# adityaX1412/Experiment-YOLO

Hardware: AMD Instinct MI355X
Metric: images/sec (train) DEAL-YOLO-N 640x640 bs=64/GPU (higher is better)
Workload: dtype f16; 1 GPU; DEAL-YOLO-N (yolov8n-ASF-P2P2.yaml) train step 640x640, per-GPU batch 64, fwd+TAL/WIOU+NWD/DFL/BCE loss+bwd+SGD+EMA, BASELINE.json configs[1]; loss_mode=wiou+nwd, settle_steps=18, capture_retries=0, global_batch=64, parallelism=dp1, hipgraph=True

## Files before the change

### experiment-yolo_amd/csrc/tensor_ops.hip

```cpp
#include <cstdlib>
#include "common.h"
#include "dealyolo_hip.h"

static inline int grid_for(long total) {
  long b = (total + 255) / 256;
  if (b > 8192) b = 8192;
  if (b < 1) b = 1;
  return (int)b;
}
static bool tensor_ops_v1() {
  const char* e = getenv("DY_TENSOR_OPS_V1");
  return e && e[0] == '1' && !e[1];
}

__global__ __launch_bounds__(256) void import_image_kernel(const float* x, f16* y, int N, int C, int H, int W, int Cp,
                                                           float mul) {
  const long hw = (long)H * W, total = (long)N * hw;
  for (long pix = (long)blockIdx.x * 256 + threadIdx.x; pix < total; pix += (long)gridDim.x * 256) {
    const long n = pix / hw, r = pix - n * hw;
    for (int c0 = 0; c0 < Cp; c0 += 8) {
      half8 v;
#pragma unroll
      for (int j = 0; j < 8; ++j) v[j] = (c0 + j < C) ? (f16)(x[(n * C + c0 + j) * hw + r] * mul) : (f16)0.f;
      *reinterpret_cast<half8*>(y + pix * Cp + c0) = v;
// ... 329 lines not shown
            bi[j] = dy * 5 + dx;
          }
        }
      }
    }
    half8 o;
    uint8_t ai[8];
#pragma unroll
    for (int j = 0; j < 8; ++j) {
      o[j] = (f16)best[j];
      ai[j] = (uint8_t)bi[j];
    }
    *reinterpret_cast<half8*>(a.y + pix * a.ldy + c0) = o;
    if (a.arg) *reinterpret_cast<uint2*>(a.arg + pix * a.C + c0) = *reinterpret_cast<uint2*>(ai);
  }
}
__global__ __launch_bounds__(256) void maxpool5_bwd_kernel(PoolArgs a) {
  const int cpp = a.C >> 3;
  const long total = (long)a.N * a.H * a.W * cpp;
  for (long idx = (long)blockIdx.x * 256 + threadIdx.x; idx < total; idx += (long)gridDim.x * 256) {
    const long pix = idx / cpp;
    const int c0 = (int)(idx - pix * cpp) * 8;
    const int x0 = (int)(pix % a.W);
    const long t = pix / a.W;
    const int y0 = (int)(t % a.H);
    const long n = t / a.H;
    float s[8];
#pragma unroll
    for (int j = 0; j < 8; ++j) s[j] = 0.f;
    if (a.accumulate) {
      const half8 o = *reinterpret_cast<const half8*>(a.y + pix * a.ldy + c0);
#pragma unroll
      for (int j = 0; j < 8; ++j) s[j] = (float)o[j];
    }
#pragma unroll
    for (int dy = 0; dy < 5; ++dy) {
      const int wy = y0 - (dy - 2);
      const bool yok = wy >= 0 && wy < a.H;
      const int yc = yok ? wy : y0;
      uint2 raw[5];
      half8 g[5];
      bool ok[5];
#pragma unroll
      for (int dx = 0; dx < 5; ++dx) {
        const int wx = x0 - (dx - 2);
        ok[dx] = yok && wx >= 0 && wx < a.W;
        const long wp = (n * a.H + yc) * a.W + (ok[dx] ? wx : x0);
        raw[dx] = *reinterpret_cast<const uint2*>(a.arg + wp * a.C + c0);
        g[dx] = *reinterpret_cast<const half8*>(a.dy + wp * a.lddy + c0);
      }
#pragma unroll
      for (int dx = 0; dx < 5; ++dx) {
        if (!ok[dx]) continue;
        const uint8_t* ai = reinterpret_cast<const uint8_t*>(&raw[dx]);
        const int code = dy * 5 + dx;
#pragma unroll
        for (int j = 0; j < 8; ++j)
          if (ai[j] == code) s[j] += (float)g[dx][j];
      }
    }
    half8 o;
#pragma unroll
    for (int j = 0; j < 8; ++j) o[j] = (f16)s[j];
    *reinterpret_cast<half8*>(a.y + pix * a.ldy + c0) = o;
  }
}
#define SPPF_THREADS 1024
struct SppfArgs {
  f16* cat;
  uint8_t* arg[3];
  int ld, C, N, H, W, acc[3];
};
template <int CG>
static __device__ __forceinline__ void sppf_pool3_fwd_body(const SppfArgs& a, char* sppf_lds) {
  constexpr int G = CG / 8;
  const int HW = a.H * a.W, items = HW * G;
  half8* cur = reinterpret_cast<half8*>(sppf_lds);
  half8* rowm = cur + items;
  uint2* rowa = reinterpret_cast<uint2*>(rowm + items);
  const int groups = a.C / CG, n = blockIdx.x / groups, c0 = (blockIdx.x - n * groups) * CG;
  f16* const base = a.cat + (size_t)n * HW * a.ld + c0;
  for (int i = threadIdx.x; i < items; i += SPPF_THREADS) {
    const int px = i / G, part = i - px * G;
    cur[i] = *reinterpret_cast<const half8*>(base + (size_t)px * a.ld + part * 8);
  }
  __syncthreads();
  for (int l = 0; l < 3; ++l) {
    for (int i = threadIdx.x; i < items; i += SPPF_THREADS) {
      const int px = i / G, part = i - px * G, y = px / a.W, x = px - y * a.W;
      float best[8];
      uint8_t bd[8];
#pragma unroll
      for (int j = 0; j < 8; ++j) { best[j] = -INFINITY; bd[j] = 0; }
#pragma unroll
      for (int dx = 0; dx < 5; ++dx) {
        const int xx = x + dx - 2;
        if (xx < 0 || xx >= a.W) continue;
        const half8 v = cur[(y * a.W + xx) * G + part];
#pragma unroll
        for (int j = 0; j < 8; ++j) {
          const float f = (float)v[j];
          if (f > best[j] || f != f) { best[j] = f; bd[j] = (uint8_t)dx; }
        }
      }
      half8 o;
#pragma unroll
      for (int j = 0; j < 8; ++j) o[j] = (f16)best[j];
      rowm[i] = o;
      rowa[i] = *reinterpret_cast<const uint2*>(bd);
    }
    __syncthreads();
    f16* const yb = base + (size_t)(l + 1) * a.C;
    uint8_t* const ab = a.arg[l] ? a.arg[l] + (size_t)n * HW * a.C + c0 : nullptr;
    for (int i = threadIdx.x; i < items; i += SPPF_THREADS) {
      const int px = i / G, part = i - px * G, y = px / a.W, x = px - y * a.W;
      float best[8];
      uint8_t bi[8];
#pragma unroll
      for (int j = 0; j < 8; ++j) { best[j] = -INFINITY; bi[j] = 0; }
#pragma unroll
      for (int dy = 0; dy < 5; ++dy) {
        const int yy = y + dy - 2;
        if (yy < 0 || yy >= a.H) continue;
        const int k = (yy * a.W + x) * G + part;
        const half8 v = rowm[k];
        const uint2 ra = rowa[k];
        const uint8_t* rd = reinterpret_cast<const uint8_t*>(&ra);
#pragma unroll
        for (int j = 0; j < 8; ++j) {
          const float f = (float)v[j];
          if (f > best[j] || f != f) { best[j] = f; bi[j] = (uint8_t)(dy * 5 + rd[j]); }
        }
      }
      half8 o;
#pragma unroll
      for (int j = 0; j < 8; ++j) o[j] = (f16)best[j];
      cur[i] = o;
      *reinterpret_cast<half8*>(yb + (size_t)px * a.ld + part * 8) = o;
      if (ab) *reinterpret_cast<uint2*>(ab + (size_t)px * a.C + part * 8) = *reinterpret_cast<const uint2*>(bi);
    }
    __syncthreads();
  }
}
template <int CG>
__global__ __launch_bounds__(SPPF_THREADS) void sppf_pool3_fwd_kernel(SppfArgs a) {
  extern __shared__ __attribute__((aligned(16))) char sppf_lds[];
  sppf_pool3_fwd_body<CG>(a, sppf_lds);
}
template <int CG>
__global__ __launch_bounds__(SPPF_THREADS) void sppf_pool3_fwd_v2_kernel(SppfArgs a) {
  constexpr int G = CG / 8;
  constexpr unsigned KNINF = 0x03ffu;
  extern __shared__ __attribute__((aligned(16))) char sppf_lds[];
  const int HW = a.H * a.W, items = HW * G;
  uint4* cur = reinterpret_cast<uint4*>(sppf_lds);
  uint4* row0 = cur + items;
  uint4* row1 = row0 + items;
  int* special = reinterpret_cast<int*>(row1 + items);
  const int groups = a.C / CG, n = blockIdx.x / groups, c0 = (blockIdx.x - n * groups) * CG;
  f16* const base = a.cat + (size_t)n * HW * a.ld + c0;
  if (threadIdx.x == 0) *special = 0;
  __syncthreads();
  bool bad = false;
  for (int i = threadIdx.x; i < items; i += SPPF_THREADS) {
    const int px = i / G, part = i - px * G;
    const uint4 v = *reinterpret_cast<const uint4*>(base + (size_t)px * a.ld + part * 8);
    const unsigned w[4] = {v.x, v.y, v.z, v.w};
    unsigned k[4];
#pragma unroll
    for (int d = 0; d < 4; ++d) {
      const unsigned lo = w[d] & 0xffffu, hi = w[d] >> 16;
      bad |= (lo & 0x7fffu) > 0x7c00u || lo == 0x8000u || (hi & 0x7fffu) > 0x7c00u || hi == 0x8000u;
      k[d] = w[d] ^ ((((w[d] >> 15) & 0x00010001u) * 0xffffu) | 0x80008000u);
    }
    cur[i] = uint4{k[0], k[1], k[2], k[3]};
  }
  if (bad) *special = 1;
  __syncthreads();
  if (*special) {
    __syncthreads();
    sppf_pool3_fwd_body<CG>(a, sppf_lds);
    return;
  }
  for (int l = 0; l < 3; ++l) {
    for (int i = threadIdx.x; i < items; i += SPPF_THREADS) {
      const int px = i / G, part = i - px * G, y = px / a.W, x = px - y * a.W;
      unsigned best[8];
#pragma unroll
      for (int dx = 0; dx < 5; ++dx) {
        const int xx = min(max(x + dx - 2, 0), a.W - 1);
        const unsigned t = (unsigned)(63 - xx);
        const uint4 v = cur[(y * a.W + xx) * G + part];
        const unsigned w[4] = {v.x, v.y, v.z, v.w};
#pragma unroll
        for (int d = 0; d < 4; ++d) {
          const unsigned lo = (w[d] << 16) | t, hi = (w[d] & 0xffff0000u) | t;
          best[2 * d] = dx ? max(best[2 * d], lo) : lo;
          best[2 * d + 1] = dx ? max(best[2 * d + 1], hi) : hi;
        }
      }
      const int kx = (63 - y) * 5 + x - 61, ninf = (63 - y) * 5 + 4;
      unsigned o[8];
#pragma unroll
      for (int j = 0; j < 8; ++j) {
        const unsigned low = (best[j] >> 16) == KNINF ? (unsigned)ninf : (unsigned)((int)(best[j] & 0xffffu) + kx);
        o[j] = (best[j] & 0xffff0000u) | low;
      }
      row0[i] = uint4{o[0], o[1], o[2], o[3]};
      row1[i] = uint4{o[4], o[5], o[6], o[7]};
    }
    __syncthreads();
    f16* const yb = base + (size_t)(l + 1) * a.C;
    uint8_t* const ab = a.arg[l] ? a.arg[l] + (size_t)n * HW * a.C + c0 : nullptr;
    for (int i = threadIdx.x; i < items; i += SPPF_THREADS) {
      const int px = i / G, part = i - px * G, y = px / a.W, x = px - y * a.W;
      unsigned best[8];
#pragma unroll
      for (int dy = 0; dy < 5; ++dy) {
        const int yy = min(max(y + dy - 2, 0), a.H - 1);
        const int k = (yy * a.W + x) * G + part;
        const uint4 v0 = row0[k], v1 = row1[k];
        const unsigned w[8] = {v0.x, v0.y, v0.z, v0.w, v1.x, v1.y, v1.z, v1.w};
#pragma unroll
        for (int j = 0; j < 8; ++j) best[j] = dy ? max(best[j], w[j]) : w[j];
      }
      const unsigned ky = (unsigned)(329 - 5 * y);
      unsigned kp[4], hv[4], code[8];
#pragma unroll
      for (int j = 0; j < 8; ++j) code[j] = (best[j] >> 16) == KNINF ? 0u : (ky - (best[j] & 0xffffu)) & 0xffu;
#pragma unroll
      for (int d = 0; d < 4; ++d) {
        kp[d] = (best[2 * d + 1] & 0xffff0000u) | (best[2 * d] >> 16);
        hv[d] = kp[d] ^ ((((~kp[d] >> 15) & 0x00010001u) * 0xffffu) | 0x80008000u);
      }
      cur[i] = uint4{kp[0], kp[1], kp[2], kp[3]};
      *reinterpret_cast<uint4*>(yb + (size_t)px * a.ld + part * 8) = uint4{hv[0], hv[1], hv[2], hv[3]};
      if (ab)
        *reinterpret_cast<uint2*>(ab + (size_t)px * a.C + part * 8) =
            uint2{code[0] | code[1] << 8 | code[2] << 16 | code[3] << 24, code[4] | code[5] << 8 | code[6] << 16 | code[7] << 24};
    }
    __syncthreads();
  }
}
template <int CG>
__global__ __launch_bounds__(SPPF_THREADS) void sppf_pool3_bwd_kernel(SppfArgs a) {
  constexpr int G = CG / 8;
  extern __shared__ __attribute__((aligned(16))) char sppf_lds[];
  const int HW = a.H * a.W, items = HW * G;
  half8* g0 = reinterpret_cast<half8*>(sppf_lds);
  half8* g1 = g0 + items;
  uint2* ar = reinterpret_cast<uint2*>(g1 + items);
  const int groups = a.C / CG, n = blockIdx.x / groups, c0 = (blockIdx.x - n * groups) * CG;
  f16* const base = a.cat + (size_t)n * HW * a.ld + c0;
  for (int i = threadIdx.x; i < items; i += SPPF_THREADS) {
    const int px = i / G, part = i - px * G;
    g0[i] = *reinterpret_cast<const half8*>(base + (size_t)3 * a.C + (size_t)px * a.ld + part * 8);
  }
  for (int l = 2; l >= 0; --l) {
    const uint8_t* const ab = a.arg[l] + (size_t)n * HW * a.C + c0;
    for (int i = threadIdx.x; i < items; i += SPPF_THREADS) {
      const int px = i / G, part = i - px * G;
      ar[i] = *reinterpret_cast<const uint2*>(ab + (size_t)px * a.C + part * 8);
    }
    __syncthreads();
    f16* const tb = base + (size_t)l * a.C;
    for (int i = threadIdx.x; i < items; i += SPPF_THREADS) {
      const int px = i / G, part = i - px * G, y = px / a.W, x = px - y * a.W;
      float s[8];
#pragma unroll
      for (int j = 0; j < 8; ++j) s[j] = 0.f;
      if (a.acc[l]) {
        const half8 o = *reinterpret_cast<const half8*>(tb + (size_t)px * a.ld + part * 8);
#pragma unroll
        for (int j = 0; j < 8; ++j) s[j] = (float)o[j];
      }
#pragma unroll
      for (int dy = 0; dy < 5; ++dy) {
        const int wy = y - (dy - 2);
        if (wy < 0 || wy >= a.H) continue;
#pragma unroll
        for (int dx = 0; dx < 5; ++dx) {
          const int wx = x - (dx - 2);
          if (wx < 0 || wx >= a.W) continue;
          const int k = (wy * a.W + wx) * G + part;
          const uint2 raw = ar[k];
          const half8 g = g0[k];
          const uint8_t* ai = reinterpret_cast<const uint8_t*>(&raw);
          const int code = dy * 5 + dx;
#pragma unroll
          for (int j = 0; j < 8; ++j)
            if (ai[j] == code) s[j] += (float)g[j];
        }
      }
      half8 o;
#pragma unroll
      for (int j = 0; j < 8; ++j) o[j] = (f16)s[j];
      if (l > 0) g1[i] = o;
      else *reinterpret_cast<half8*>(tb + (size_t)px * a.ld + part * 8) = o;
    }
    __syncthreads();
    half8* t = g0; g0 = g1; g1 = t;
  }
}
extern "C" int dy_sppf_pool3_supported(int h, int w, int C) {
  if (h < 1 || w < 1 || C < 8 || (C & 7)) return 0;
  const long px = (long)h * w;
  if (!(C & 15) && px * (2 * 32 + 16) <= 156 * 1024) return 16;
  if (px * (2 * 16 + 8) <= 156 * 1024) return 8;
  return 0;
}
extern "C" int dy_sppf_pool3(void* cat, int ld, int C, void* arg0, void* arg1, void* arg2, int n, int h, int w, hipStream_t stream) {
  const int cg = dy_sppf_pool3_supported(h, w, C);
  if (!cg || !cat || ld < 4 * C) return DY_ERR_ARG;
  if ((ld & 7) || ((uintptr_t)cat & 15)) return DY_ERR_ALIGN;
  SppfArgs a{(f16*)cat, {(uint8_t*)arg0, (uint8_t*)arg1, (uint8_t*)arg2}, ld, C, n, h, w, {0, 0, 0}};
  const size_t lds2 = (size_t)h * w * (cg / 8) * 48 + 16;
  if (!tensor_ops_v1() && h <= 63 && w <= 63 && lds2 <= 156 * 1024) {
    static bool attr2[2] = {false, false};
    if (cg == 16) {
      if (!attr2[0]) { if (hipFuncSetAttribute(reinterpret_cast<const void*>(sppf_pool3_fwd_v2_kernel<16>), hipFuncAttributeMaxDynamicSharedMemorySize, 156 * 1024) != hipSuccess) return DY_ERR_LAUNCH; attr2[0] = true; }
      hipLaunchKernelGGL(sppf_pool3_fwd_v2_kernel<16>, dim3(n * (C / 16)), dim3(SPPF_THREADS), lds2, stream, a);
    } else {
      if (!attr2[1]) { if (hipFuncSetAttribute(reinterpret_cast<const void*>(sppf_pool3_fwd_v2_kernel<8>), hipFuncAttributeMaxDynamicSharedMemorySize, 156 * 1024) != hipSuccess) return DY_ERR_LAUNCH; attr2[1] = true; }
      hipLaunchKernelGGL(sppf_pool3_fwd_v2_kernel<8>, dim3(n * (C / 8)), dim3(SPPF_THREADS), lds2, stream, a);
    }
    DY_CHECK_LAUNCH();
    return DY_OK;
  }
  const size_t lds = (size_t)h * w * (cg / 8) * (2 * 16 + 8);
  static bool attr[2] = {false, false};
  if (cg == 16) {
    if (!attr[0]) { if (hipFuncSetAttribute(reinterpret_cast<const void*>(sppf_pool3_fwd_kernel<16>), hipFuncAttributeMaxDynamicSharedMemorySize, 156 * 1024) != hipSuccess) return DY_ERR_LAUNCH; attr[0] = true; }
    hipLaunchKernelGGL(sppf_pool3_fwd_kernel<16>, dim3(n * (C / 16)), dim3(SPPF_THREADS), lds, stream, a);
  } else {
    if (!attr[1]) { if (hipFuncSetAttribute(reinterpret_cast<const void*>(sppf_pool3_fwd_kernel<8>), hipFuncAttributeMaxDynamicSharedMemorySize, 156 * 1024) != hipSuccess) return DY_ERR_LAUNCH; attr[1] = true; }
    hipLaunchKernelGGL(sppf_pool3_fwd_kernel<8>, dim3(n * (C / 8)), dim3(SPPF_THREADS), lds, stream, a);
  }
  DY_CHECK_LAUNCH();
  return DY_OK;
}
extern "C" int dy_sppf_pool3_backward(void* gcat, int ld, int C, const void* arg0, const void* arg1, const void* arg2, int n, int h,
                                      int w, int acc0, int acc1, int acc2, hipStream_t stream) {
  const int cg = dy_sppf_pool3_supported(h, w, C);
  if (!cg || !gcat || !arg0 || !arg1 || !arg2 || ld < 4 * C) return DY_ERR_ARG;
  if ((ld & 7) || ((uintptr_t)gcat & 15)) return DY_ERR_ALIGN;
  SppfArgs a{(f16*)gcat, {(uint8_t*)arg0, (uint8_t*)arg1, (uint8_t*)arg2}, ld, C, n, h, w, {acc0, acc1, acc2}};
  const size_t lds = (size_t)h * w * (cg / 8) * (2 * 16 + 8);
  static bool attr[2] = {false, false};
  if (cg == 16) {
    if (!attr[0]) { if (hipFuncSetAttribute(reinterpret_cast<const void*>(sppf_pool3_bwd_kernel<16>), hipFuncAttributeMaxDynamicSharedMemorySize, 156 * 1024) != hipSuccess) return DY_ERR_LAUNCH; attr[0] = true; }
    hipLaunchKernelGGL(sppf_pool3_bwd_kernel<16>, dim3(n * (C / 16)), dim3(SPPF_THREADS), lds, stream, a);
  } else {
    if (!attr[1]) { if (hipFuncSetAttribute(reinterpret_cast<const void*>(sppf_pool3_bwd_kernel<8>), hipFuncAttributeMaxDynamicSharedMemorySize, 156 * 1024) != hipSuccess) return DY_ERR_LAUNCH; attr[1] = true; }
    hipLaunchKernelGGL(sppf_pool3_bwd_kernel<8>, dim3(n * (C / 8)), dim3(SPPF_THREADS), lds, stream, a);
  }
  DY_CHECK_LAUNCH();
  return DY_OK;
}

extern "C" int dy_maxpool5(const void* x, int ldx, void* y, int ldy, void* argmax, int n, int h, int w, int C,
                           hipStream_t stream) {
  if ((C & 7) || (ldx & 7) || (ldy & 7)) return DY_ERR_ALIGN;
  PoolArgs a{(const f16*)x, (f16*)y, (uint8_t*)argmax, nullptr, ldx, ldy, 0, C, n, h, w, 0};
  hipLaunchKernelGGL(maxpool5_fwd_kernel, dim3(grid_for((long)n * h * w * (C >> 3))), dim3(256), 0, stream, a);
  DY_CHECK_LAUNCH();
  return DY_OK;
}
extern "C" int dy_maxpool5_backward(const void* dy, int lddy, const void* argmax, void* dx, int lddx, int n, int h,
                                    int w, int C, int accumulate, hipStream_t stream) {
  if ((C & 7) || (lddy & 7) || (lddx & 7)) return DY_ERR_ALIGN;
  PoolArgs a{nullptr, (f16*)dx, (uint8_t*)argmax, (const f16*)dy, 0, lddx, lddy, C, n, h, w, accumulate};
  hipLaunchKernelGGL(maxpool5_bwd_kernel, dim3(grid_for((long)n * h * w * (C >> 3))), dim3(256), 0, stream, a);
  DY_CHECK_LAUNCH();
  return DY_OK;
}

struct SsArgs {
  const f16* r[3];
  int ld[3];
  const f16* res;
  int ldres;
  f16* y;
  int ldy;
  const float* coef;
  int C, N, H, W;
};
__global__ __launch_bounds__(256) void scalseq_tail_kernel(SsArgs a) {
  const int cpp = a.C >> 3;
  const long total = (long)a.N * a.H * a.W * cpp;
  for (long idx = (long)blockIdx.x * 256 + threadIdx.x; idx < total; idx += (long)gridDim.x * 256) {
    const long pix = idx / cpp;
    const int c0 = (int)(idx - pix * cpp) * 8;
    const int x0 = (int)(pix % a.W);
    const long t = pix / a.W;
    const int y0 = (int)(t % a.H);
    const long n = t / a.H;
    float best[8];
#pragma unroll
    for (int l = 0; l < 3; ++l) {
      const int hl = a.H >> l, wl = a.W >> l;
      const long src = (n * hl + (y0 >> l)) * wl + (x0 >> l);
      const half8 v = *reinterpret_cast<const half8*>(a.r[l] + src * a.ld[l] + c0);
#pragma unroll
      for (int j = 0; j < 8; ++j) {
        float z = (float)v[j] * a.coef[c0 + j] + a.coef[a.C + c0 + j];
        z = z > 0.f ? z : 0.1f * z;
        if (l == 0 || z > best[j] || z != z) best[j] = z;
      }
    }
    half8 o;
    if (a.res) {
      const half8 rv = *reinterpret_cast<const half8*>(a.res + pix * a.ldres + c0);
#pragma unroll
      for (int j = 0; j < 8; ++j) best[j] = (float)(f16)best[j] + (float)rv[j];
    }
#pragma unroll
    for (int j = 0; j < 8; ++j) o[j] = (f16)best[j];
    *reinterpret_cast<half8*>(a.y + pix * a.ldy + c0) = o;
  }
}
extern "C" int dy_scalseq_tail(const void* r0, int ld0, const void* r1, int ld1, const void* r2, int ld2,
                               const void* res, int ldres, void* y, int ldy, const float* coef, int n, int h, int w,
                               int C, hipStream_t stream) {
  if ((C & 7) || (ld0 & 7) || (ld1 & 7) || (ld2 & 7) || (ldy & 7) || (h & 3) || (w & 3)) return DY_ERR_ALIGN;
  SsArgs a{{(const f16*)r0, (const f16*)r1, (const f16*)r2}, {ld0, ld1, ld2}, (const f16*)res, ldres, (f16*)y, ldy,
           coef, C, n, h, w};
  hipLaunchKernelGGL(scalseq_tail_kernel, dim3(grid_for((long)n * h * w * (C >> 3))), dim3(256), 0, stream, a);
  DY_CHECK_LAUNCH();
  return DY_OK;
}

struct SsBwdArgs {
  const f16* r[3];
  int ld[3];
  const f16* dy;
  int lddy;
  f16* dr;
  int lddr;
  const float* coef;
  const float* bwdcoef;
  float* partials;
  int C, N, H, W, level, mode;
};
__global__ __launch_bounds__(256) void scalseq_bwd_kernel(SsBwdArgs a) {
  const int cpp = a.C >> 3, l = a.level, s = 1 << l;
  const int hl = a.H >> l, wl = a.W >> l;
  const long total = (long)a.N * hl * wl * cpp;
  float ps[8], px[8];
#pragma unroll
  for (int j = 0; j < 8; ++j) ps[j] = px[j] = 0.f;
  const int part = threadIdx.x % cpp, c0 = part * 8;
  const int rows = 256 / cpp, row = threadIdx.x / cpp;
  const long npix_l = (long)a.N * hl * wl;
  if (row < rows) {
    for (long lp = (long)blockIdx.x * rows + row; lp < npix_l; lp += (long)gridDim.x * rows) {
      const int lx = (int)(lp % wl);
      const long t = lp / wl;
      const int ly = (int)(t % hl);
      const long n = t / hl;
      const half8 own = *reinterpret_cast<const half8*>(a.r[l] + lp * a.ld[l] + c0);
      float gsum[8];
#pragma unroll
      for (int j = 0; j < 8; ++j) gsum[j] = 0.f;
      for (int i = 0; i < s * s; ++i) {
        const int y0 = ly * s + i / s, x0 = lx * s + i % s;
        const long pos = (n * a.H + y0) * a.W + x0;
        const half8 g = *reinterpret_cast<const half8*>(a.dy + pos * a.lddy + c0);
        half8 v[3];
#pragma unroll
        for (int k = 0; k < 3; ++k) {
          if (k == l) {
            v[k] = own;
          } else {
            const int hk = a.H >> k, wk = a.W >> k;
            v[k] = *reinterpret_cast<const half8*>(a.r[k] + ((n * hk + (y0 >> k)) * wk + (x0 >> k)) * a.ld[k] + c0);
          }
        }
#pragma unroll
        for (int j = 0; j < 8; ++j) {
          const float sc = a.coef[c0 + j], sh = a.coef[a.C + c0 + j];
          float z[3];
#pragma unroll
          for (int k = 0; k < 3; ++k) {
            const float zz = (float)v[k][j] * sc + sh;
            z[k] = zz > 0.f ? zz : 0.1f * zz;
          }
          int am = 0;
          if (z[1] > z[am]) am = 1;
          if (z[2] > z[am]) am = 2;
          if (am == l) {
            const float zz = (float)own[j] * sc + sh;
            gsum[j] += (float)g[j] * (zz > 0.f ? 1.f : 0.1f);
          }
        }
      }
      if (a.mode == 0) {
#pragma unroll
        for (int j = 0; j < 8; ++j) {
          const float xh = ((float)own[j] - a.coef[2 * a.C + c0 + j]) * a.coef[3 * a.C + c0 + j];
          ps[j] += gsum[j];
          px[j] += gsum[j] * xh;
        }
      } else {
        half8 o;
        const float cnt = (float)(s * s);
#pragma unroll
        for (int j = 0; j < 8; ++j) {
          const float xh = ((float)own[j] - a.coef[2 * a.C + c0 + j]) * a.coef[3 * a.C + c0 + j];
          o[j] = (f16)(a.coef[c0 + j] * (gsum[j] - cnt * a.bwdcoef[c0 + j] - cnt * xh * a.bwdcoef[a.C + c0 + j]));
        }
        *reinterpret_cast<half8*>(a.dr + lp * a.lddr + c0) = o;
      }
    }
  }
  if (a.mode == 0) {
    __shared__ float red[2][256][9];
#pragma unroll
    for (int j = 0; j < 8; ++j) {
      red[0][threadIdx.x][j] = ps[j];
      red[1][threadIdx.x][j] = px[j];
    }
    __syncthreads();
    for (int i = threadIdx.x; i < 2 * a.C; i += 256) {
      const int which = i / a.C, c = i - which * a.C, pp = c >> 3, j = c & 7;
      float sum = 0.f;
      for (int r = 0; r < rows; ++r) sum += red[which][r * cpp + pp][j];
      a.partials[((size_t)blockIdx.x * 2 + which) * a.C + c] = sum;
    }
  }
  (void)total;
}
extern "C" int dy_scalseq_tail_backward(const void* r0, int ld0, const void* r1, int ld1, const void* r2, int ld2,
                                        const void* dy, int lddy, void* dr, int lddr, const float* coef,
                                        const float* bwdcoef, float* partials, int max_partials, int n, int h, int w,
                                        int C, int level, int mode, int* nparts, hipStream_t stream) {
  if ((C & 7) || (C >> 3) > 256 || (h & 3) || (w & 3) || level < 0 || level > 2) return DY_ERR_ARG;
  SsBwdArgs a{{(const f16*)r0, (const f16*)r1, (const f16*)r2}, {ld0, ld1, ld2}, (const f16*)dy, lddy, (f16*)dr, lddr,
              coef, bwdcoef, partials, C, n, h, w, level, mode};
  const int rows = 256 / (C >> 3);
  long blocks = ((long)n * (h >> level) * (w >> level) + rows - 1) / rows;
  if (blocks > 1024) blocks = 1024;
  if (mode == 0 && blocks > max_partials) blocks = max_partials;
  if (blocks < 1) blocks = 1;
  if (nparts) *nparts = (int)blocks;
  hipLaunchKernelGGL(scalseq_bwd_kernel, dim3((int)blocks), dim3(256), 0, stream, a);
  DY_CHECK_LAUNCH();
  return DY_OK;
}

struct SsBwdAllArgs {
  const f16* r[3];
  int ld[3];
  const f16* dy;
  int lddy;
  f16* dr[3];
  int lddr[3];
  const float* coef;
  const float* bwdcoef;
  float* partials;
  int C, N, H, W, mode;
};
__global__ __launch_bounds__(256) void scalseq_bwd_all_kernel(SsBwdAllArgs a) {
  const int cpp = a.C >> 3;
  const int h1 = a.H >> 1, w1 = a.W >> 1, h2 = a.H >> 2, w2 = a.W >> 2;
  const int part = threadIdx.x % cpp, c0 = part * 8;
  const int rows = 256 / cpp, row = threadIdx.x / cpp;
  const long npix2 = (long)a.N * h2 * w2;
  float sc[8], sh[8], mean[8], inv[8], mg[8], mgx[8], ps[8], px[8];
#pragma unroll
  for (int j = 0; j < 8; ++j) {
    sc[j] = a.coef[c0 + j];
    sh[j] = a.coef[a.C + c0 + j];
    mean[j] = a.coef[2 * a.C + c0 + j];
    inv[j] = a.coef[3 * a.C + c0 + j];
    mg[j] = a.mode ? a.bwdcoef[c0 + j] : 0.f;
    mgx[j] = a.mode ? a.bwdcoef[a.C + c0 + j] : 0.f;
    ps[j] = px[j] = 0.f;
  }
  if (row < rows) {
    for (long lp2 = (long)blockIdx.x * rows + row; lp2 < npix2; lp2 += (long)gridDim.x * rows) {
      const int lx2 = (int)(lp2 % w2);
      const long t = lp2 / w2;
      const int ly2 = (int)(t % h2);
      const long n = t / h2;
      const half8 own2 = *reinterpret_cast<const half8*>(a.r[2] + lp2 * a.ld[2] + c0);
      float z2[8], gs2[8];
#pragma unroll
      for (int j = 0; j < 8; ++j) {
        const float zz = (float)own2[j] * sc[j] + sh[j];
        z2[j] = zz > 0.f ? zz : 0.1f * zz;
        gs2[j] = 0.f;
      }
      for (int q1 = 0; q1 < 4; ++q1) {
        const int ly1 = ly2 * 2 + (q1 >> 1), lx1 = lx2 * 2 + (q1 & 1);
        const long lp1 = (n * h1 + ly1) * w1 + lx1;
        const half8 own1 = *reinterpret_cast<const half8*>(a.r[1] + lp1 * a.ld[1] + c0);
        float z1[8], gs1[8];
#pragma unroll
        for (int j = 0; j < 8; ++j) {
          const float zz = (float)own1[j] * sc[j] + sh[j];
          z1[j] = zz > 0.f ? zz : 0.1f * zz;
          gs1[j] = 0.f;
        }
#pragma unroll
        for (int q0 = 0; q0 < 4; ++q0) {
          const int y0 = ly1 * 2 + (q0 >> 1), x0 = lx1 * 2 + (q0 & 1);
          const long pos = (n * a.H + y0) * a.W + x0;
          const half8 own0 = *reinterpret_cast<const half8*>(a.r[0] + pos * a.ld[0] + c0);
          const half8 g = *reinterpret_cast<const half8*>(a.dy + pos * a.lddy + c0);
          half8 o;
#pragma unroll
          for (int j = 0; j < 8; ++j) {
            const float zz0 = (float)own0[j] * sc[j] + sh[j];
            const float z0 = zz0 > 0.f ? zz0 : 0.1f * zz0;
            int am = 0;
            float zb = z0;
            if (z1[j] > zb) { am = 1; zb = z1[j]; }
            if (z2[j] > zb) { am = 2; zb = z2[j]; }
            const float gg = (float)g[j] * (zb > 0.f ? 1.f : 0.1f);
            const float g0 = am == 0 ? gg : 0.f;
            gs1[j] += am == 1 ? gg : 0.f;
            gs2[j] += am == 2 ? gg : 0.f;
            const float xh0 = ((float)own0[j] - mean[j]) * inv[j];
            if (a.mode == 0) {
              ps[j] += g0;
              px[j] += g0 * xh0;
            } else {
              o[j] = (f16)(sc[j] * (g0 - mg[j] - xh0 * mgx[j]));
            }
          }
          if (a.mode) *reinterpret_cast<half8*>(a.dr[0] + pos * a.lddr[0] + c0) = o;
        }
        half8 o1;
#pragma unroll
        for (int j = 0; j < 8; ++j) {
          const float xh = ((float)own1[j] - mean[j]) * inv[j];
          if (a.mode == 0) {
            ps[j] += gs1[j];
            px[j] += gs1[j] * xh;
          } else {
            o1[j] = (f16)(sc[j] * (gs1[j] - 4.f * mg[j] - 4.f * xh * mgx[j]));
          }
        }
        if (a.mode) *reinterpret_cast<half8*>(a.dr[1] + lp1 * a.lddr[1] + c0) = o1;
      }
      half8 o2;
#pragma unroll
      for (int j = 0; j < 8; ++j) {
        const float xh = ((float)own2[j] - mean[j]) * inv[j];
        if (a.mode == 0) {
          ps[j] += gs2[j];
          px[j] += gs2[j] * xh;
        } else {
          o2[j] = (f16)(sc[j] * (gs2[j] - 16.f * mg[j] - 16.f * xh * mgx[j]));
        }
      }
      if (a.mode) *reinterpret_cast<half8*>(a.dr[2] + lp2 * a.lddr[2] + c0) = o2;
    }
  }
  if (a.mode == 0) {
    __shared__ float red[2][256][9];
#pragma unroll
    for (int j = 0; j < 8; ++j) {
      red[0][threadIdx.x][j] = ps[j];
      red[1][threadIdx.x][j] = px[j];
    }
    __syncthreads();
    for (int i = threadIdx.x; i < 2 * a.C; i += 256) {
      const int which = i / a.C, c = i - which * a.C, pp = c >> 3, j = c & 7;
      float sum = 0.f;
      for (int r = 0; r < rows; ++r) sum += red[which][r * cpp + pp][j];
      a.partials[((size_t)blockIdx.x * 2 + which) * a.C + c] = sum;
    }
  }
}
__global__ __launch_bounds__(256) void scalseq_bwd_cols_kernel(SsBwdAllArgs a) {
  const int cpp = a.C >> 3, PW = 64 / cpp;
  const int h1 = a.H >> 1, w1 = a.W >> 1, h2 = a.H >> 2, w2 = a.W >> 2;
  const int tid = threadIdx.x, wave = tid >> 6, lane = tid & 63;
  const int part = lane % cpp, col = lane / cpp, c0 = part * 8;
  float sc[8], sh[8], mean[8], inv[8], mg[8], mgx[8], ps[8], px[8];
#pragma unroll
  for (int j = 0; j < 8; ++j) {
    sc[j] = a.coef[c0 + j];
    sh[j] = a.coef[a.C + c0 + j];
    mean[j] = a.coef[2 * a.C + c0 + j];
    inv[j] = a.coef[3 * a.C + c0 + j];
    mg[j] = a.mode ? a.bwdcoef[c0 + j] : 0.f;
    mgx[j] = a.mode ? a.bwdcoef[a.C + c0 + j] : 0.f;
    ps[j] = px[j] = 0.f;
  }
  const int chunks = a.W / PW;
  const long items = (long)a.N * h2 * chunks;
  for (long it = (long)blockIdx.x * 4 + wave; it < items; it += (long)gridDim.x * 4) {
    const int xc = (int)(it % chunks);
    const long t = it / chunks;
    const int y2 = (int)(t % h2);
    const long n = t / h2;
    const int x = xc * PW + col;
    const long lp2 = (n * h2 + y2) * w2 + (x >> 2);
    const half8 own2 = *reinterpret_cast<const half8*>(a.r[2] + lp2 * a.ld[2] + c0);
    float z2[8], gs2[8];
#pragma unroll
    for (int j = 0; j < 8; ++j) {
      const float zz = (float)own2[j] * sc[j] + sh[j];
      z2[j] = zz > 0.f ? zz : 0.1f * zz;
      gs2[j] = 0.f;
    }
#pragma unroll
    for (int hf = 0; hf < 2; ++hf) {
      const int y1 = y2 * 2 + hf;
      const long lp1 = (n * h1 + y1) * w1 + (x >> 1);
      const half8 own1 = *reinterpret_cast<const half8*>(a.r[1] + lp1 * a.ld[1] + c0);
      float z1[8], gs1[8];
#pragma unroll
      for (int j = 0; j < 8; ++j) {
        const float zz = (float)own1[j] * sc[j] + sh[j];
        z1[j] = zz > 0.f ? zz : 0.1f * zz;
        gs1[j] = 0.f;
      }
#pragma unroll
      for (int rr = 0; rr < 2; ++rr) {
        const long pos = (n * a.H + (y1 * 2 + rr)) * a.W + x;
        const half8 own0 = *reinterpret_cast<const half8*>(a.r[0] + pos * a.ld[0] + c0);
        const half8 g = *reinterpret_cast<const half8*>(a.dy + pos * a.lddy + c0);
        half8 o;
#pragma unroll
        for (int j = 0; j < 8; ++j) {
          const float zz0 = (float)own0[j] * sc[j] + sh[j];
          const float z0 = zz0 > 0.f ? zz0 : 0.1f * zz0;
          int am = 0;
          float zb = z0;
          if (z1[j] > zb) { am = 1; zb = z1[j]; }
          if (z2[j] > zb) { am = 2; zb = z2[j]; }
          const float gg = (float)g[j] * (zb > 0.f ? 1.f : 0.1f);
          const float g0 = am == 0 ? gg : 0.f;
          gs1[j] += am == 1 ? gg : 0.f;
          gs2[j] += am == 2 ? gg : 0.f;
          const float xh0 = ((float)own0[j] - mean[j]) * inv[j];
          if (a.mode == 0) {
            ps[j] += g0;
            px[j] += g0 * xh0;
          } else {
            o[j] = (f16)(sc[j] * (g0 - mg[j] - xh0 * mgx[j]));
          }
        }
        if (a.mode) *reinterpret_cast<half8*>(a.dr[0] + pos * a.lddr[0] + c0) = o;
      }
      half8 o1;
#pragma unroll
      for (int j = 0; j < 8; ++j) {
        const float tot = gs1[j] + (cpp == 4 ? dpp_read<DY_DPP_ROW_SHL(4)>(gs1[j]) : __shfl_xor(gs1[j], cpp, 64));
        const float xh = ((float)own1[j] - mean[j]) * inv[j];
        if (a.mode == 0) {
          if (!(col & 1)) { ps[j] += tot; px[j] += tot * xh; }
        } else {
          o1[j] = (f16)(sc[j] * (tot - 4.f * mg[j] - 4.f * xh * mgx[j]));
        }
      }
      if (a.mode && !(col & 1)) *reinterpret_cast<half8*>(a.dr[1] + lp1 * a.lddr[1] + c0) = o1;
    }
    half8 o2;
#pragma unroll
    for (int j = 0; j < 8; ++j) {
      float tot;
      if (cpp == 4) {
        tot = gs2[j] + dpp_read<DY_DPP_ROW_SHL(4)>(gs2[j]);
        tot += dpp_read<DY_DPP_ROW_SHL(8)>(tot);
      } else {
        tot = gs2[j] + __shfl_xor(gs2[j], cpp, 64);
        tot += __shfl_xor(tot, 2 * cpp, 64);
      }
      const float xh = ((float)own2[j] - mean[j]) * inv[j];
      if (a.mode == 0) {
        if (!(col & 3)) { ps[j] += tot; px[j] += tot * xh; }
      } else {
        o2[j] = (f16)(sc[j] * (tot - 16.f * mg[j] - 16.f * xh * mgx[j]));
      }
    }
    if (a.mode && !(col & 3)) *reinterpret_cast<half8*>(a.dr[2] + lp2 * a.lddr[2] + c0) = o2;
  }
  if (a.mode == 0) {
    __shared__ float red[2][256][9];
    const int rows = 256 / cpp;
#pragma unroll
    for (int j = 0; j < 8; ++j) {
      red[0][tid][j] = ps[j];
      red[1][tid][j] = px[j];
    }
    __syncthreads();
    for (int i = tid; i < 2 * a.C; i += 256) {
      const int which = i / a.C, c = i - which * a.C, pp = c >> 3, j = c & 7;
      float sum = 0.f;
      for (int r = 0; r < rows; ++r) sum += red[which][r * cpp + pp][j];
      a.partials[((size_t)blockIdx.x * 2 + which) * a.C + c] = sum;
    }
  }
}
static __device__ __forceinline__ half8 ld16(const f16* sbase, unsigned voff) {
  return *reinterpret_cast<const half8*>(reinterpret_cast<const char*>(sbase) + voff);
}
static __device__ __forceinline__ void st16(f16* sbase, unsigned voff, uint4 v) {
  *reinterpret_cast<uint4*>(reinterpret_cast<char*>(sbase) + voff) = v;
}
static __device__ __forceinline__ void mul_to_f16(int hi, unsigned& pk, float a, float b) {
  if (hi) asm("v_fma_mixhi_f16 %0, %1, %2, 0" : "+v"(pk) : "v"(a), "v"(b));
  else asm("v_fma_mixlo_f16 %0, %1, %2, 0" : "+v"(pk) : "v"(a), "v"(b));
}
template <int CPP, int MODE>
__global__ __launch_bounds__(256, 4) void scalseq_bwd_v2_kernel(SsBwdAllArgs a, int nvb) {
#pragma clang fp contract(off)
  constexpr int PW = 64 / CPP, ROWS = 256 / CPP, CC = CPP * 8;
  const int h1 = a.H >> 1, w1 = a.W >> 1, h2 = a.H >> 2, w2 = a.W >> 2;
  const int tid = threadIdx.x, lane = tid & 63;
  const int wave = __builtin_amdgcn_readfirstlane(tid >> 6);
  const int part = lane % CPP, col = lane / CPP, c0 = part * 8;
  __shared__ float cf[6][CC];
  if (tid < CC) {
#pragma unroll
    for (int k = 0; k < 4; ++k) cf[k][tid] = a.coef[k * CC + tid];
    cf[4][tid] = MODE ? a.bwdcoef[tid] : 0.f;
    cf[5][tid] = MODE ? a.bwdcoef[CC + tid] : 0.f;
  }
  __syncthreads();
  float ps[8], px[8];
  const unsigned vo0 = (unsigned)(col * a.ld[0] + c0) * 2u, vody = (unsigned)(col * a.lddy + c0) * 2u;
  const unsigned vo1 = (unsigned)((col >> 1) * a.ld[1] + c0) * 2u, vo2 = (unsigned)((col >> 2) * a.ld[2] + c0) * 2u;
  const unsigned vd0 = MODE ? (unsigned)(col * a.lddr[0] + c0) * 2u : 0u, vd1 = MODE ? (unsigned)((col >> 1) * a.lddr[1] + c0) * 2u : 0u;
  const unsigned vd2 = MODE ? (unsigned)((col >> 2) * a.lddr[2] + c0) * 2u : 0u;
  const unsigned chunks = (unsigned)(a.W / PW);
  const unsigned items = (unsigned)a.N * (unsigned)h2 * chunks;
  const unsigned nv = MODE ? gridDim.x : (unsigned)nvb;
  __shared__ float red[MODE ? 1 : 2][MODE ? 1 : 256][9];
  for (unsigned vb = blockIdx.x; vb < nv; vb += gridDim.x) {
#pragma unroll
    for (int j = 0; j < 8; ++j) ps[j] = px[j] = 0.f;
    for (unsigned it = vb * 4 + (unsigned)wave; it < items; it += nv * 4) {
      const unsigned xc = it % chunks, t = it / chunks;
      const int y2 = (int)(t % (unsigned)h2);
      const long n = (long)(t / (unsigned)h2);
      const long x0 = (long)(xc * PW);
      const long lp2 = (n * h2 + y2) * w2 + (x0 >> 2);
      long lp1[2], pos[4];
      half8 own2, own1[2], own0[4], g[4];
      unsigned pk0[4][4] = {}, pk1[2][4] = {}, pk2[4] = {};
      int coff = c0;
      asm volatile("" : "+v"(coff));
      const float* const cp = &cf[0][0] + coff;
      float sc[8], sh[8], mean[8], inv[8], mg[8], mgx[8];
#pragma unroll
      for (int j = 0; j < 8; ++j) {
        sc[j] = cp[j]; sh[j] = cp[CC + j]; mean[j] = cp[2 * CC + j]; inv[j] = cp[3 * CC + j];
        mg[j] = MODE ? cp[4 * CC + j] : 0.f; mgx[j] = MODE ? cp[5 * CC + j] : 0.f;
      }
      own2 = ld16(a.r[2] + lp2 * a.ld[2], vo2);
#pragma unroll
      for (int hf = 0; hf < 2; ++hf) {
        lp1[hf] = (n * h1 + (y2 * 2 + hf)) * w1 + (x0 >> 1);
        own1[hf] = ld16(a.r[1] + lp1[hf] * a.ld[1], vo1);
      }
#pragma unroll
      for (int q = 0; q < 4; ++q) {
        pos[q] = (n * a.H + (y2 * 4 + q)) * a.W + x0;
        own0[q] = ld16(a.r[0] + pos[q] * a.ld[0], vo0);
        g[q] = ld16(a.dy + pos[q] * a.lddy, vody);
      }
      asm volatile("" : "+v"(own2), "+v"(own1[0]), "+v"(own1[1]), "+v"(own0[0]), "+v"(own0[1]), "+v"(own0[2]), "+v"(own0[3]), "+v"(g[0]), "+v"(g[1]),
                        "+v"(g[2]), "+v"(g[3]));
#pragma unroll
      for (int j = 0; j < 8; ++j) {
        const float zz2 = __builtin_fmaf((float)own2[j], sc[j], sh[j]);
        const float z2 = zz2 > 0.f ? zz2 : 0.1f * zz2;
        float gs2 = 0.f;
#pragma unroll
        for (int hf = 0; hf < 2; ++hf) {
          const float zz1 = __builtin_fmaf((float)own1[hf][j], sc[j], sh[j]);
          const float z1 = zz1 > 0.f ? zz1 : 0.1f * zz1;
          float gs1 = 0.f;
#pragma unroll
          for (int rr = 0; rr < 2; ++rr) {
            const int q = hf * 2 + rr;
            const float zz0 = __builtin_fmaf((float)own0[q][j], sc[j], sh[j]);
            const float z0 = zz0 > 0.f ? zz0 : 0.1f * zz0;
            int am = 0;
            float zb = z0;
            if (z1 > zb) { am = 1; zb = z1; }
            if (z2 > zb) { am = 2; zb = z2; }
            const float gg = (float)g[q][j] * (zb > 0.f ? 1.f : 0.1f);
            const float g0 = am == 0 ? gg : 0.f;
            gs1 += am == 1 ? gg : 0.f;
            gs2 += am == 2 ? gg : 0.f;
            const float xh0 = ((float)own0[q][j] - mean[j]) * inv[j];
            if (MODE == 0) {
              ps[j] += g0;
              px[j] = __builtin_fmaf(xh0, g0, px[j]);
            } else {
              mul_to_f16(j & 1, pk0[q][j >> 1], sc[j], __builtin_fmaf(-mgx[j], xh0, g0 - mg[j]));
            }
          }
          const float tot = gs1 + (CPP == 4 ? dpp_read<DY_DPP_ROW_SHL(4)>(gs1) : __shfl_xor(gs1, CPP, 64));
          const float xh = ((float)own1[hf][j] - mean[j]) * inv[j];
          if (MODE == 0) {
            if (!(col & 1)) { ps[j] += tot; px[j] = __builtin_fmaf(xh, tot, px[j]); }
          } else {
            mul_to_f16(j & 1, pk1[hf][j >> 1], sc[j], __builtin_fmaf(mgx[j], -4.f * xh, tot - 4.f * mg[j]));
          }
        }
        float tot;
        if (CPP == 4) {
          tot = gs2 + dpp_read<DY_DPP_ROW_SHL(4)>(gs2);
          tot += dpp_read<DY_DPP_ROW_SHL(8)>(tot);
        } else {
          tot = gs2 + __shfl_xor(gs2, CPP, 64);
          tot += __shfl_xor(tot, 2 * CPP, 64);
        }
        const float xh = ((float)own2[j] - mean[j]) * inv[j];
        if (MODE == 0) {
          if (!(col & 3)) { ps[j] += tot; px[j] = __builtin_fmaf(xh, tot, px[j]); }
        } else {
          mul_to_f16(j & 1, pk2[j >> 1], sc[j], __builtin_fmaf(mgx[j], -16.f * xh, tot - 16.f * mg[j]));
        }
      }
      if (MODE) {
#pragma unroll
        for (int q = 0; q < 4; ++q) st16(a.dr[0] + pos[q] * a.lddr[0], vd0, uint4{pk0[q][0], pk0[q][1], pk0[q][2], pk0[q][3]});
        if (!(col & 1)) {
#pragma unroll
          for (int hf = 0; hf < 2; ++hf) st16(a.dr[1] + lp1[hf] * a.lddr[1], vd1, uint4{pk1[hf][0], pk1[hf][1], pk1[hf][2], pk1[hf][3]});
        }
        if (!(col & 3)) st16(a.dr[2] + lp2 * a.lddr[2], vd2, uint4{pk2[0], pk2[1], pk2[2], pk2[3]});
      }
    }
    if constexpr (MODE == 0) {
#pragma unroll
      for (int j = 0; j < 8; ++j) {
        red[0][tid][j] = ps[j];
        red[1][tid][j] = px[j];
      }
      __syncthreads();
      if (tid < 2 * CC) {
        const int which = tid / CC, c = tid - which * CC, pp = c >> 3, j = c & 7;
        float sum = 0.f;
#pragma unroll 16
        for (int r = 0; r < ROWS; ++r) sum += red[which][r * CPP + pp][j];
        a.partials[((size_t)vb * 2 + which) * CC + c] = sum;
      }
      __syncthreads();
    }
  }
}
static int g_scalseq_grid_cap = 0;
extern "C" int dy_scalseq_bwd_grid_cap(int cap) {
  const int old = g_scalseq_grid_cap;
  g_scalseq_grid_cap = cap > 0 ? cap : 0;
  return old;
}
template <int CPP>
static void scalseq_v2_launch(const SsBwdAllArgs& a, int mode, int nvb, int grid, hipStream_t stream) {
  if (mode) hipLaunchKernelGGL((scalseq_bwd_v2_kernel<CPP, 1>), dim3(grid), dim3(256), 0, stream, a, nvb);
  else hipLaunchKernelGGL((scalseq_bwd_v2_kernel<CPP, 0>), dim3(grid), dim3(256), 0, stream, a, nvb);
}
extern "C" int dy_scalseq_tail_backward_all(const void* r0, int ld0, const void* r1, int ld1, const void* r2, int ld2,
                                            const void* dy, int lddy, void* dr0, int lddr0, void* dr1, int lddr1,
                                            void* dr2, int lddr2, const float* coef, const float* bwdcoef,
                                            float* partials, int max_partials, int n, int h, int w, int C, int mode,
                                            int* nparts, hipStream_t stream) {
  if ((C & 7) || (C >> 3) > 256 || (h & 3) || (w & 3) || (ld0 & 7) || (ld1 & 7) || (ld2 & 7) || (lddy & 7)) return DY_ERR_ARG;
  if (mode && ((lddr0 & 7) || (lddr1 & 7) || (lddr2 & 7) || !dr0 || !dr1 || !dr2 || !bwdcoef)) return DY_ERR_ARG;
  if (!mode && !partials) return DY_ERR_ARG;
  SsBwdAllArgs a{{(const f16*)r0, (const f16*)r1, (const f16*)r2}, {ld0, ld1, ld2}, (const f16*)dy, lddy,
                 {(f16*)dr0, (f16*)dr1, (f16*)dr2}, {lddr0, lddr1, lddr2}, coef, bwdcoef, partials, C, n, h, w, mode};
  const int rows = 256 / (C >> 3);
  long blocks = ((long)n * (h >> 2) * (w >> 2) + rows - 1) / rows;
  if (blocks > 2048) blocks = 2048;
  if (mode == 0 && blocks > max_partials) blocks = max_partials;
  if (blocks < 1) blocks = 1;
  const int cpp = C >> 3;
  if (cpp <= 16 && 64 % cpp == 0 && w % (64 / cpp) == 0) {
    long wblocks = ((long)n * (h >> 2) * (w / (64 / cpp)) + 3) / 4;
    if (wblocks > 2048) wblocks = 2048;
    if (mode == 0 && wblocks > max_partials) wblocks = max_partials;
    if (wblocks < 1) wblocks = 1;
    if (nparts) *nparts = (int)wblocks;
    const long items = (long)n * (h >> 2) * (w / (64 / cpp));
    if (!tensor_ops_v1() && items < (1L << 31) - 4 * 2048) {
      const int cap = g_scalseq_grid_cap ? g_scalseq_grid_cap : DY_NUM_CUS * 4;
      const int grid = wblocks < cap ? (int)wblocks : cap;
      switch (cpp) {
        case 1: scalseq_v2_launch<1>(a, mode, (int)wblocks, grid, stream); break;
        case 2: scalseq_v2_launch<2>(a, mode, (int)wblocks, grid, stream); break;
        case 4: scalseq_v2_launch<4>(a, mode, (int)wblocks, grid, stream); break;
        case 8: scalseq_v2_launch<8>(a, mode, (int)wblocks, grid, stream); break;
        default: scalseq_v2_launch<16>(a, mode, (int)wblocks, grid, stream); break;
      }
      DY_CHECK_LAUNCH();
      return DY_OK;
    }
    hipLaunchKernelGGL(scalseq_bwd_cols_kernel, dim3((int)wblocks), dim3(256), 0, stream, a);
    DY_CHECK_LAUNCH();
    return DY_OK;
  }
  if (nparts) *nparts = (int)blocks;
  hipLaunchKernelGGL(scalseq_bwd_all_kernel, dim3((int)blocks), dim3(256), 0, stream, a);
  DY_CHECK_LAUNCH();
  return DY_OK;
}

__global__ __launch_bounds__(256) void copy_slice_kernel(EwArgs e) {
  const int cpp = e.C >> 3;
  const long total = e.npix * cpp;
  for (long idx = (long)blockIdx.x * 256 + threadIdx.x; idx < total; idx += (long)gridDim.x * 256) {
    const long pix = idx / cpp;
    const int c0 = (int)(idx - pix * cpp) * 8;
    *reinterpret_cast<uint4*>(e.y + pix * e.ldy + c0) = *reinterpret_cast<const uint4*>(e.a + pix * e.lda + c0);
  }
}
extern "C" int dy_copy_slice(const void* x, int ldx, void* y, int ldy, long npix, int C, hipStream_t stream) {
  if ((C & 7) || (ldx & 7) || (ldy & 7)) return DY_ERR_ALIGN;
  EwArgs e{(const f16*)x, nullptr, nullptr, (f16*)y, ldx, 0, 0, ldy, C, npix};
  hipLaunchKernelGGL(copy_slice_kernel, dim3(grid_for(npix * (C >> 3))), dim3(256), 0, stream, e);
  DY_CHECK_LAUNCH();
  return DY_OK;
}
extern "C" int dy_fill_zero(void* p, size_t bytes, hipStream_t stream) {
  return hipMemsetAsync(p, 0, bytes, stream) == hipSuccess ? DY_OK : DY_ERR_LAUNCH;
}

struct ZpArgs {
  const f16* x;
  f16* y;
  const f16* dy;
  f16* dx;
  int ldx, ldy, lddy, lddx, C, N, H, W, accumulate;
};
__global__ __launch_bounds__(256) void zoom_pool_fwd_kernel(ZpArgs a) {
  const int cpp = a.C >> 3;
  const long total = (long)a.N * a.H * a.W * cpp;
  for (long idx = (long)blockIdx.x * 256 + threadIdx.x; idx < total; idx += (long)gridDim.x * 256) {
    const long pix = idx / cpp;
    const int c0 = (int)(idx - pix * cpp) * 8;
    const int ox = (int)(pix % a.W);
    const long t = pix / a.W;
    const int oy = (int)(t % a.H);
    const long n = t / a.H;
    float mx[8], sm[8];
#pragma unroll
    for (int i = 0; i < 4; ++i) {
      const long src = (n * 2 * a.H + 2 * oy + (i >> 1)) * 2 * a.W + 2 * ox + (i & 1);
      const half8 v = *reinterpret_cast<const half8*>(a.x + src * a.ldx + c0);
#pragma unroll
      for (int j = 0; j < 8; ++j) {
        const float f = (float)v[j];
        mx[j] = i == 0 ? f : fmaxf(mx[j], f);
        sm[j] = i == 0 ? f : sm[j] + f;
      }
    }
    half8 o;
#pragma unroll
    for (int j = 0; j < 8; ++j) o[j] = (f16)((float)(f16)mx[j] + (float)(f16)(sm[j] * 0.25f));
    *reinterpret_cast<half8*>(a.y + pix * a.ldy + c0) = o;
  }
}
__global__ __launch_bounds__(256) void zoom_pool_bwd_kernel(ZpArgs a) {
  const int cpp = a.C >> 3;
  const long total = (long)a.N * a.H * a.W * cpp;
  for (long idx = (long)blockIdx.x * 256 + threadIdx.x; idx < total; idx += (long)gridDim.x * 256) {
    const long pix = idx / cpp;
    const int c0 = (int)(idx - pix * cpp) * 8;
    const int ox = (int)(pix % a.W);
    const long t = pix / a.W;
    const int oy = (int)(t % a.H);
    const long n = t / a.H;
    const half8 g = *reinterpret_cast<const half8*>(a.dy + pix * a.lddy + c0);
    half8 v[4];
    long src[4];
#pragma unroll
    for (int i = 0; i < 4; ++i) {
      src[i] = (n * 2 * a.H + 2 * oy + (i >> 1)) * 2 * a.W + 2 * ox + (i & 1);
      v[i] = *reinterpret_cast<const half8*>(a.x + src[i] * a.ldx + c0);
    }
    int am[8];
#pragma unroll
    for (int j = 0; j < 8; ++j) {
      am[j] = 0;
      float best = (float)v[0][j];
#pragma unroll
      for (int i = 1; i < 4; ++i)
        if ((float)v[i][j] > best) {
          best = (float)v[i][j];
          am[j] = i;
        }
    }
#pragma unroll
    for (int i = 0; i < 4; ++i) {
      f16* d = a.dx + src[i] * a.lddx + c0;
      half8 o;
      if (a.accumulate) o = *reinterpret_cast<const half8*>(d);
#pragma unroll
      for (int j = 0; j < 8; ++j) {
        const float gi = (float)g[j] * (0.25f + (am[j] == i ? 1.f : 0.f));
        o[j] = (f16)(gi + (a.accumulate ? (float)o[j] : 0.f));
      }
      *reinterpret_cast<half8*>(d) = o;
    }
  }
}
extern "C" int dy_zoom_pool(const void* x, int ldx, void* y, int ldy, int n, int h, int w, int C, hipStream_t stream) {
  if ((C & 7) || (ldx & 7) || (ldy & 7)) return DY_ERR_ALIGN;
  ZpArgs a{(const f16*)x, (f16*)y, nullptr, nullptr, ldx, ldy, 0, 0, C, n, h, w, 0};
  hipLaunchKernelGGL(zoom_pool_fwd_kernel, dim3(grid_for((long)n * h * w * (C >> 3))), dim3(256), 0, stream, a);
  DY_CHECK_LAUNCH();
  return DY_OK;
}
extern "C" int dy_zoom_pool_backward(const void* x, int ldx, const void* dy, int lddy, void* dx, int lddx, int n, int h,
                                     int w, int C, int accumulate, hipStream_t stream) {
  if ((C & 7) || (ldx & 7) || (lddy & 7) || (lddx & 7)) return DY_ERR_ALIGN;
  ZpArgs a{(const f16*)x, nullptr, (const f16*)dy, (f16*)dx, ldx, 0, lddy, lddx, C, n, h, w, accumulate};
  hipLaunchKernelGGL(zoom_pool_bwd_kernel, dim3(grid_for((long)n * h * w * (C >> 3))), dim3(256), 0, stream, a);
  DY_CHECK_LAUNCH();
  return DY_OK;
}
```

Measured before the change: 6175 images/s.

## Add padded-LDS SPPF pool backward kernel and retune scalseq bwd occupancy

Adds a new SPPF 5x5 maxpool backward kernel that keeps the gradient and argmax planes in a zero-padded LDS tile. Border checks disappear, the next level's argmax and accumulation values are prefetched into registers, and the per-tap argmax compare-and-add uses packed bit tricks and mixed-precision FMA. This is meant to cut branchy per-tap work and global round trips in the pooling backward pass. Separately, the scalseq backward MODE=1 kernel drops its launch-bounds occupancy target from 4 to 3 waves per SIMD and caps its grid to match, giving it more registers at the cost of fewer resident blocks.

```diff
diff --git a/experiment-yolo_amd/csrc/tensor_ops.hip b/experiment-yolo_amd/csrc/tensor_ops.hip
--- a/experiment-yolo_amd/csrc/tensor_ops.hip
+++ b/experiment-yolo_amd/csrc/tensor_ops.hip
@@ -655,6 +655,140 @@
     half8* t = g0; g0 = g1; g1 = t;
   }
 }
+static __device__ __forceinline__ void sppf_mix_add_lo(float& s, const unsigned v) {
+  asm("v_fma_mix_f32 %0, %1, 1.0, %0 op_sel_hi:[1,0,0]" : "+v"(s) : "v"(v));
+}
+static __device__ __forceinline__ void sppf_mix_add_hi(float& s, const unsigned v) {
+  asm("v_fma_mix_f32 %0, %1, 1.0, %0 op_sel:[1,0,0] op_sel_hi:[1,0,0]" : "+v"(s) : "v"(v));
+}
+static __device__ __forceinline__ unsigned sppf_differs(const unsigned a, const unsigned cw, const unsigned k7f) {
+  unsigned t;
+  asm("v_xad_u32 %0, %1, %2, %3" : "=v"(t) : "v"(a), "s"(cw), "v"(k7f));
+  return t;
+}
+static __device__ __forceinline__ unsigned sppf_addend(const unsigned m, const unsigned g) {
+  unsigned v;
+  asm("v_bfi_b32 %0, %1, %2, %3" : "=v"(v) : "v"(m), "s"(0x80008000u), "v"(g));
+  return v;
+}
+static __device__ __forceinline__ void sppf_tap8(float (&s)[8], const uint2 a, const uint4 g, const unsigned cw, const unsigned k7f) {
+  const unsigned aw[2] = {a.x, a.y}, gw[4] = {g.x, g.y, g.z, g.w};
+#pragma unroll
+  for (int d = 0; d < 2; ++d) {
+    const unsigned t = sppf_differs(aw[d], cw, k7f), u = t << 8;
+    const unsigned v01 = sppf_addend(__builtin_amdgcn_perm(t, u, 0x0b0b0a0au), gw[2 * d]);
+    const unsigned v23 = sppf_addend(__builtin_amdgcn_perm(t, u, 0x09090808u), gw[2 * d + 1]);
+    sppf_mix_add_lo(s[4 * d], v01);
+    sppf_mix_add_hi(s[4 * d + 1], v01);
+    sppf_mix_add_lo(s[4 * d + 2], v23);
+    sppf_mix_add_hi(s[4 * d + 3], v23);
+  }
+}
+static __device__ __forceinline__ unsigned sppf_stage_arg(const unsigned r) {
+  const unsigned v = (r | ((r & 0x80808080u) >> 1)) & 0x7f7f7f7fu;
+  return __builtin_amdgcn_perm(v, v, 0x01030002u);
+}
+#define SPPF_BWD2_ITEMS 4
+template <int CG>
+__global__ __launch_bounds__(SPPF_THREADS) void sppf_pool3_bwd_v2_kernel(SppfArgs a) {
+  constexpr int G = CG / 8;
+  extern __shared__ __attribute__((aligned(16))) char sppf_lds[];
+  const int HW = a.H * a.W, items = HW * G, PW = a.W + 4, P = (a.H + 4) * PW * G;
+  uint4* gin = reinterpret_cast<uint4*>(sppf_lds);
+  uint4* gout = gin + P;
+  uint2* ar = reinterpret_cast<uint2*>(gout + P);
+  const int groups = a.C / CG, n = blockIdx.x / groups, c0 = (blockIdx.x - n * groups) * CG;
+  f16* const base = a.cat + (size_t)n * HW * a.ld + c0;
+  const size_t abase = (size_t)n * HW * a.C + c0;
+  const uint8_t* const arg0 = a.arg[0] + abase;
+  const uint8_t* const arg1 = a.arg[1] + abase;
+  const uint8_t* const arg2 = a.arg[2] + abase;
+  const int acc0 = a.acc[0], acc1 = a.acc[1], acc2 = a.acc[2];
+  for (int q = threadIdx.x; q < P; q += SPPF_THREADS) {
+    const int pp = q / G, part = q - pp * G, py = pp / PW - 2, px = pp - (py + 2) * PW - 2;
+    if (py >= 0 && py < a.H && px >= 0 && px < a.W) {
+      gin[q] = *reinterpret_cast<const uint4*>(base + (size_t)3 * a.C + (size_t)(py * a.W + px) * a.ld + part * 8);
+    } else {
+      gin[q] = uint4{0u, 0u, 0u, 0u};
+      gout[q] = uint4{0u, 0u, 0u, 0u};
+      ar[q] = uint2{0x7f7f7f7fu, 0x7f7f7f7fu};
+    }
+  }
+  int qi[SPPF_BWD2_ITEMS];
+  uint2 parg[SPPF_BWD2_ITEMS];
+  uint4 pacc[SPPF_BWD2_ITEMS];
+#pragma unroll
+  for (int k = 0; k < SPPF_BWD2_ITEMS; ++k) {
+    const int i = threadIdx.x + k * SPPF_THREADS, px = i / G, part = i - px * G, y = px / a.W, x = px - y * a.W;
+    qi[k] = ((y + 2) * PW + x + 2) * G + part;
+    parg[k] = uint2{0u, 0u};
+    pacc[k] = uint4{0u, 0u, 0u, 0u};
+    if (i < items) {
+      parg[k] = *reinterpret_cast<const uint2*>(arg2 + (size_t)px * a.C + part * 8);
+      if (acc2) pacc[k] = *reinterpret_cast<const uint4*>(base + (size_t)2 * a.C + (size_t)px * a.ld + part * 8);
+    }
+  }
+#pragma unroll 1
+  for (int l = 2; l >= 0; --l) {
+#pragma unroll
+    for (int k = 0; k < SPPF_BWD2_ITEMS; ++k) {
+      if (threadIdx.x + k * SPPF_THREADS < items) {
+        ar[qi[k]] = uint2{sppf_stage_arg(parg[k].x), sppf_stage_arg(parg[k].y)};
+        gout[qi[k]] = pacc[k];
+      }
+    }
+    __syncthreads();
+    if (l > 0) {
+      const uint8_t* const ab = l == 2 ? arg1 : arg0;
+      const int accn = l == 2 ? acc1 : acc0;
+      const f16* const tbn = base + (size_t)(l - 1) * a.C;
+#pragma unroll
+      for (int k = 0; k < SPPF_BWD2_ITEMS; ++k) {
+        const int i = threadIdx.x + k * SPPF_THREADS, px = i / G, part = i - px * G;
+        pacc[k] = uint4{0u, 0u, 0u, 0u};
+        if (i < items) {
+          parg[k] = *reinterpret_cast<const uint2*>(ab + (size_t)px * a.C + part * 8);
+          if (accn) pacc[k] = *reinterpret_cast<const uint4*>(tbn + (size_t)px * a.ld + part * 8);
+        }
+      }
+    }
+    const int rowq = PW * G;
+    const unsigned k7f = 0x7f7f7f7fu;
+#pragma unroll 1
+    for (int i = threadIdx.x; i < items; i += SPPF_THREADS) {
+      const int px = i / G, part = i - px * G, y = px / a.W, x = px - y * a.W;
+      const int q = ((y + 2) * PW + x + 2) * G + part;
+      const half8 o0 = *reinterpret_cast<const half8*>(gout + q);
+      float s[8];
+#pragma unroll
+      for (int j = 0; j < 8; ++j) s[j] = (float)o0[j];
+      uint2 ta[2][5];
+      uint4 tg[2][5];
+#pragma unroll
+      for (int dy = -1; dy < 5; ++dy) {
+        if (dy < 4) {
+          const int qr = q - (dy - 1) * rowq - 2 * G;
+#pragma unroll
+          for (int dx = 0; dx < 5; ++dx) {
+            ta[(dy + 1) & 1][dx] = ar[qr + (4 - dx) * G];
+            tg[(dy + 1) & 1][dx] = gin[qr + (4 - dx) * G];
+          }
+        }
+        if (dy >= 0) {
+#pragma unroll
+          for (int dx = 0; dx < 5; ++dx) sppf_tap8(s, ta[dy & 1][dx], tg[dy & 1][dx], (unsigned)(dy * 5 + dx) * 0x01010101u, k7f);
+        }
+      }
+      half8 o;
+#pragma unroll
+      for (int j = 0; j < 8; ++j) o[j] = (f16)s[j];
+      if (l > 0) *reinterpret_cast<half8*>(gout + q) = o;
+      else *reinterpret_cast<half8*>(base + (size_t)px * a.ld + part * 8) = o;
+    }
+    __syncthreads();
+    uint4* t = gin; gin = gout; gout = t;
+  }
+}
 extern "C" int dy_sppf_pool3_supported(int h, int w, int C) {
   if (h < 1 || w < 1 || C < 8 || (C & 7)) return 0;
   const long px = (long)h * w;
@@ -698,6 +832,19 @@
   if (!cg || !gcat || !arg0 || !arg1 || !arg2 || ld < 4 * C) return DY_ERR_ARG;
   if ((ld & 7) || ((uintptr_t)gcat & 15)) return DY_ERR_ALIGN;
   SppfArgs a{(f16*)gcat, {(uint8_t*)arg0, (uint8_t*)arg1, (uint8_t*)arg2}, ld, C, n, h, w, {acc0, acc1, acc2}};
+  const size_t lds2 = (size_t)(h + 4) * (w + 4) * (cg / 8) * (2 * 16 + 8);
+  if (!tensor_ops_v1() && lds2 <= 156 * 1024 && (long)h * w * (cg / 8) <= SPPF_BWD2_ITEMS * SPPF_THREADS) {
+    static bool attr2[2] = {false, false};
+    if (cg == 16) {
+      if (!attr2[0]) { if (hipFuncSetAttribute(reinterpret_cast<const void*>(sppf_pool3_bwd_v2_kernel<16>), hipFuncAttributeMaxDynamicSharedMemorySize, 156 * 1024) != hipSuccess) return DY_ERR_LAUNCH; attr2[0] = true; }
+      hipLaunchKernelGGL(sppf_pool3_bwd_v2_kernel<16>, dim3(n * (C / 16)), dim3(SPPF_THREADS), lds2, stream, a);
+    } else {
+      if (!attr2[1]) { if (hipFuncSetAttribute(reinterpret_cast<const void*>(sppf_pool3_bwd_v2_kernel<8>), hipFuncAttributeMaxDynamicSharedMemorySize, 156 * 1024) != hipSuccess) return DY_ERR_LAUNCH; attr2[1] = true; }
+      hipLaunchKernelGGL(sppf_pool3_bwd_v2_kernel<8>, dim3(n * (C / 8)), dim3(SPPF_THREADS), lds2, stream, a);
+    }
+    DY_CHECK_LAUNCH();
+    return DY_OK;
+  }
   const size_t lds = (size_t)h * w * (cg / 8) * (2 * 16 + 8);
   static bool attr[2] = {false, false};
   if (cg == 16) {
@@ -1161,7 +1308,7 @@
   else asm("v_fma_mixlo_f16 %0, %1, %2, 0" : "+v"(pk) : "v"(a), "v"(b));
 }
 template <int CPP, int MODE>
-__global__ __launch_bounds__(256, 4) void scalseq_bwd_v2_kernel(SsBwdAllArgs a, int nvb) {
+__global__ __launch_bounds__(256, MODE ? 3 : 4) void scalseq_bwd_v2_kernel(SsBwdAllArgs a, int nvb) {
 #pragma clang fp contract(off)
   constexpr int PW = 64 / CPP, ROWS = 256 / CPP, CC = CPP * 8;
   const int h1 = a.H >> 1, w1 = a.W >> 1, h2 = a.H >> 2, w2 = a.W >> 2;
@@ -1337,7 +1484,7 @@
     if (nparts) *nparts = (int)wblocks;
     const long items = (long)n * (h >> 2) * (w / (64 / cpp));
     if (!tensor_ops_v1() && items < (1L << 31) - 4 * 2048) {
-      const int cap = g_scalseq_grid_cap ? g_scalseq_grid_cap : DY_NUM_CUS * 4;
+      const int cap = g_scalseq_grid_cap ? g_scalseq_grid_cap : DY_NUM_CUS * (mode ? 3 : 4);
       const int grid = wblocks < cap ? (int)wblocks : cap;
       switch (cpp) {
         case 1: scalseq_v2_launch<1>(a, mode, (int)wblocks, grid, stream); break;
```

New measurement: 6213 images/s, median of 6. Within noise of the previous version (+0.6%).
